# gmweir/PYFFT

Measured on AMD Instinct MI355X. Metric: Msamples/sec Welch-PSD 4096-pt Hann 50% overlap, complex64, higher is better.
Workload: dtype f32

## Files before the change

### pyfft_amd/csrc/fft_core.h

```cpp
#pragma once
#include <type_traits>
#include <hip/hip_runtime.h>

namespace sp {

typedef float2 cf;

__device__ __forceinline__ cf mk(float a, float b) { return make_float2(a, b); }
__device__ __forceinline__ cf operator+(cf a, cf b) { return mk(a.x + b.x, a.y + b.y); }
__device__ __forceinline__ cf operator-(cf a, cf b) { return mk(a.x - b.x, a.y - b.y); }
__device__ __forceinline__ cf operator*(float s, cf a) { return mk(s * a.x, s * a.y); }
__device__ __forceinline__ cf cmul(cf a, cf b) { return mk(a.x * b.x - a.y * b.y, a.x * b.y + a.y * b.x); }
__device__ __forceinline__ cf cmulc(cf a, cf b) { return mk(a.x * b.x + a.y * b.y, a.y * b.x - a.x * b.y); }
__device__ __forceinline__ cf cconj(cf a) { return mk(a.x, -a.y); }
__device__ __forceinline__ float cnorm(cf a) { return a.x * a.x + a.y * a.y; }

template <bool INV> __device__ __forceinline__ cf rot(cf a) { return INV ? mk(-a.y, a.x) : mk(a.y, -a.x); }
template <bool INV> __device__ __forceinline__ cf twc(cf a, float C, float S) {
    return INV ? mk(a.x * C - a.y * S, a.y * C + a.x * S) : mk(a.x * C + a.y * S, a.y * C - a.x * S);
}
template <bool INV> __device__ __forceinline__ cf twm(cf a, cf w) { return INV ? cmulc(a, w) : cmul(a, w); }

#define SP_C8 0.70710678118654752440f
#define SP_C16 0.92387953251128675613f
#define SP_S16 0.38268343236508977173f

template <bool INV> __device__ __forceinline__ void dft2(cf &a, cf &b) {
    cf t = a - b;
    a = a + b;
    b = t;
}

template <bool INV> __device__ __forceinline__ void dft4(cf &a, cf &b, cf &c, cf &d) {
    cf t0 = a + c, t1 = a - c, t2 = b + d, t3 = rot<INV>(b - d);
    a = t0 + t2;
    c = t0 - t2;
    b = t1 + t3;
    d = t1 - t3;
}

template <bool INV> __device__ __forceinline__ void dft8(cf (&x)[8]) {
    dft4<INV>(x[0], x[2], x[4], x[6]);
    dft4<INV>(x[1], x[3], x[5], x[7]);
    cf o1 = twc<INV>(x[3], SP_C8, SP_C8);
    cf o2 = rot<INV>(x[5]);
    cf o3 = twc<INV>(x[7], -SP_C8, SP_C8);
    cf e0 = x[0], e1 = x[2], e2 = x[4], e3 = x[6], o0 = x[1];
    x[0] = e0 + o0;
    x[4] = e0 - o0;
    x[1] = e1 + o1;
    x[5] = e1 - o1;
    x[2] = e2 + o2;
    x[6] = e2 - o2;
    x[3] = e3 + o3;
    x[7] = e3 - o3;
}

template <bool INV> __device__ __forceinline__ void dft16(cf (&x)[16]) {
#pragma unroll
    for (int b = 0; b < 4; ++b) dft4<INV>(x[b], x[b + 4], x[b + 8], x[b + 12]);
    x[5] = twc<INV>(x[5], SP_C16, SP_S16);
    x[9] = twc<INV>(x[9], SP_C8, SP_C8);
    x[13] = twc<INV>(x[13], SP_S16, SP_C16);
    x[6] = twc<INV>(x[6], SP_C8, SP_C8);
    x[10] = rot<INV>(x[10]);
    x[14] = twc<INV>(x[14], -SP_C8, SP_C8);
    x[7] = twc<INV>(x[7], SP_S16, SP_C16);
    x[11] = twc<INV>(x[11], -SP_C8, SP_C8);
    x[15] = twc<INV>(x[15], -SP_C16, -SP_S16);
#pragma unroll
    for (int c = 0; c < 4; ++c) dft4<INV>(x[4 * c], x[4 * c + 1], x[4 * c + 2], x[4 * c + 3]);
    cf t;
#define SP_SWAP(i, j) t = x[i]; x[i] = x[j]; x[j] = t;
    SP_SWAP(1, 4) SP_SWAP(2, 8) SP_SWAP(3, 12) SP_SWAP(6, 9) SP_SWAP(7, 13) SP_SWAP(11, 14)
#undef SP_SWAP
}

struct Tw16 {
    float f[40];
    static constexpr int TAU = 0, RB = 15, RC = 19, RD = 23, S1 = 27, S2 = 31, S3 = 35;
};

#define SP_T16 0.41421356237309504880f
#define SP_T316 2.41421356237309504880f

__device__ __forceinline__ void dft4s(cf &a, cf &b, cf &c, cf &d, float rb, float rc, float rd) {
    const cf t0 = mk(fmaf(rc, c.x, a.x), fmaf(rc, c.y, a.y));
    const cf t1 = mk(fmaf(-rc, c.x, a.x), fmaf(-rc, c.y, a.y));
    const cf t2 = mk(fmaf(rd, d.x, b.x), fmaf(rd, d.y, b.y));
    const cf t3 = mk(fmaf(-rd, d.x, b.x), fmaf(-rd, d.y, b.y));
    a = mk(fmaf(rb, t2.x, t0.x), fmaf(rb, t2.y, t0.y));
    c = mk(fmaf(-rb, t2.x, t0.x), fmaf(-rb, t2.y, t0.y));
    b = mk(fmaf(rb, t3.y, t1.x), fmaf(-rb, t3.x, t1.y));
    d = mk(fmaf(-rb, t3.y, t1.x), fmaf(rb, t3.x, t1.y));
}
__device__ __forceinline__ cf rot_tan(cf a, float t) { return mk(fmaf(t, a.y, a.x), fmaf(-t, a.x, a.y)); }

template <bool TWD, bool PREROT = false> __device__ __forceinline__ void dft16s(cf (&x)[16], const Tw16 &w) {
    if constexpr (TWD) {
        if constexpr (!PREROT) {
#pragma unroll
            for (int s = 1; s < 16; ++s) x[s] = rot_tan(x[s], w.f[Tw16::TAU + s - 1]);
        }
#pragma unroll
        for (int b = 0; b < 4; ++b) dft4s(x[b], x[b + 4], x[b + 8], x[b + 12], w.f[Tw16::RB + b], w.f[Tw16::RC + b], w.f[Tw16::RD + b]);
    } else {
#pragma unroll
        for (int b = 0; b < 4; ++b) dft4<false>(x[b], x[b + 4], x[b + 8], x[b + 12]);
    }
    x[5] = rot_tan(x[5], SP_T16);
    x[9] = mk(x[9].x + x[9].y, x[9].y - x[9].x);
    x[13] = rot_tan(x[13], SP_T316);
    x[6] = mk(x[6].x + x[6].y, x[6].y - x[6].x);
    x[10] = mk(x[10].y, -x[10].x);
    x[14] = mk(x[14].x - x[14].y, x[14].y + x[14].x);
    x[7] = rot_tan(x[7], SP_T316);
    x[11] = mk(x[11].x - x[11].y, x[11].y + x[11].x);
    x[15] = rot_tan(x[15], SP_T16);
    if constexpr (TWD) {
#pragma unroll
        for (int c = 0; c < 4; ++c) dft4s(x[4 * c], x[4 * c + 1], x[4 * c + 2], x[4 * c + 3], w.f[Tw16::S1 + c], w.f[Tw16::S2 + c], w.f[Tw16::S3 + c]);
    } else {
        dft4<false>(x[0], x[1], x[2], x[3]);
        dft4s(x[4], x[5], x[6], x[7], SP_C16, SP_C8, SP_S16 / SP_C16);
        dft4s(x[8], x[9], x[10], x[11], SP_C8, 1.f, -1.f);
        dft4s(x[12], x[13], x[14], x[15], SP_S16, -SP_C8, -SP_C16 / SP_S16);
    }
    cf t;
#define SP_SWAP(i, j) t = x[i]; x[i] = x[j]; x[j] = t;
    SP_SWAP(1, 4) SP_SWAP(2, 8) SP_SWAP(3, 12) SP_SWAP(6, 9) SP_SWAP(7, 13) SP_SWAP(11, 14)
#undef SP_SWAP
}

template <bool TWD, class Store, bool PREROT = false> __device__ __forceinline__ void dft16s_es(cf (&x)[16], const Tw16 &w, Store store) {
    if constexpr (TWD) {
        if constexpr (!PREROT) {
#pragma unroll
            for (int s = 1; s < 16; ++s) x[s] = rot_tan(x[s], w.f[Tw16::TAU + s - 1]);
        }
#pragma unroll
        for (int b = 0; b < 4; ++b) dft4s(x[b], x[b + 4], x[b + 8], x[b + 12], w.f[Tw16::RB + b], w.f[Tw16::RC + b], w.f[Tw16::RD + b]);
    } else {
#pragma unroll
        for (int b = 0; b < 4; ++b) dft4<false>(x[b], x[b + 4], x[b + 8], x[b + 12]);
    }
    x[5] = rot_tan(x[5], SP_T16);
    x[9] = mk(x[9].x + x[9].y, x[9].y - x[9].x);
    x[13] = rot_tan(x[13], SP_T316);
    x[6] = mk(x[6].x + x[6].y, x[6].y - x[6].x);
    x[10] = mk(x[10].y, -x[10].x);
    x[14] = mk(x[14].x - x[14].y, x[14].y + x[14].x);
    x[7] = rot_tan(x[7], SP_T316);
    x[11] = mk(x[11].x - x[11].y, x[11].y + x[11].x);
    x[15] = rot_tan(x[15], SP_T16);
    __builtin_amdgcn_sched_barrier(0);
#define SP_ES_OUT(c)                                                                                                 \
    store(c, x[4 * c]);                                                                                              \
    store(c + 4, x[4 * c + 1]);                                                                                      \
    store(c + 8, x[4 * c + 2]);                                                                                      \
    store(c + 12, x[4 * c + 3]);                                                                                     \
    __builtin_amdgcn_sched_barrier(0);
    if constexpr (TWD) {
        dft4s(x[0], x[1], x[2], x[3], w.f[Tw16::S1 + 0], w.f[Tw16::S2 + 0], w.f[Tw16::S3 + 0]);
        SP_ES_OUT(0)
        dft4s(x[4], x[5], x[6], x[7], w.f[Tw16::S1 + 1], w.f[Tw16::S2 + 1], w.f[Tw16::S3 + 1]);
        SP_ES_OUT(1)
        dft4s(x[8], x[9], x[10], x[11], w.f[Tw16::S1 + 2], w.f[Tw16::S2 + 2], w.f[Tw16::S3 + 2]);
        SP_ES_OUT(2)
        dft4s(x[12], x[13], x[14], x[15], w.f[Tw16::S1 + 3], w.f[Tw16::S2 + 3], w.f[Tw16::S3 + 3]);
        SP_ES_OUT(3)
    } else {
        dft4<false>(x[0], x[1], x[2], x[3]);
        SP_ES_OUT(0)
        dft4s(x[4], x[5], x[6], x[7], SP_C16, SP_C8, SP_S16 / SP_C16);
        SP_ES_OUT(1)
        dft4s(x[8], x[9], x[10], x[11], SP_C8, 1.f, -1.f);
        SP_ES_OUT(2)
        dft4s(x[12], x[13], x[14], x[15], SP_S16, -SP_C8, -SP_C16 / SP_S16);
        SP_ES_OUT(3)
    }
#undef SP_ES_OUT
}

__device__ __forceinline__ void dft4w(cf &a, cf &b, cf &c, cf &d, float wa, float wb, float wc, float wd) {
    const cf pa = mk(wa * a.x, wa * a.y), pb = mk(wb * b.x, wb * b.y);
    const cf t0 = mk(fmaf(wc, c.x, pa.x), fmaf(wc, c.y, pa.y));
    const cf t1 = mk(fmaf(-wc, c.x, pa.x), fmaf(-wc, c.y, pa.y));
    const cf t2 = mk(fmaf(wd, d.x, pb.x), fmaf(wd, d.y, pb.y));
    const cf t3 = mk(fmaf(-wd, d.x, pb.x), fmaf(-wd, d.y, pb.y));
    a = t0 + t2;
    c = t0 - t2;
    b = mk(t1.x + t3.y, t1.y - t3.x);
    d = mk(t1.x - t3.y, t1.y + t3.x);
}
struct NoMid {
    __device__ __forceinline__ void operator()(int) const {}
};
template <class Store, class Mid = NoMid> __device__ __forceinline__ void dft16s_es_win(cf (&x)[16], const float (&w)[16], Store store, Mid mid = Mid()) {
#pragma unroll
    for (int b = 0; b < 4; ++b) {
        dft4w(x[b], x[b + 4], x[b + 8], x[b + 12], w[b], w[b + 4], w[b + 8], w[b + 12]);
        if constexpr (!std::is_same<Mid, NoMid>::value) {
            if (b < 3) {
                __builtin_amdgcn_sched_barrier(0);
                mid(b);
                __builtin_amdgcn_sched_barrier(0);
            }
        }
    }
    x[5] = rot_tan(x[5], SP_T16);
    x[9] = mk(x[9].x + x[9].y, x[9].y - x[9].x);
    x[13] = rot_tan(x[13], SP_T316);
    x[6] = mk(x[6].x + x[6].y, x[6].y - x[6].x);
    x[10] = mk(x[10].y, -x[10].x);
    x[14] = mk(x[14].x - x[14].y, x[14].y + x[14].x);
    x[7] = rot_tan(x[7], SP_T316);
    x[11] = mk(x[11].x - x[11].y, x[11].y + x[11].x);
    x[15] = rot_tan(x[15], SP_T16);
    __builtin_amdgcn_sched_barrier(0);
#define SP_ES_OUT(c)                                                                                                 \
    store(c, x[4 * c]);                                                                                              \
    store(c + 4, x[4 * c + 1]);                                                                                      \
    store(c + 8, x[4 * c + 2]);                                                                                      \
    store(c + 12, x[4 * c + 3]);                                                                                     \
    __builtin_amdgcn_sched_barrier(0);
    dft4<false>(x[0], x[1], x[2], x[3]);
    SP_ES_OUT(0)
    dft4s(x[4], x[5], x[6], x[7], SP_C16, SP_C8, SP_S16 / SP_C16);
    SP_ES_OUT(1)
    dft4s(x[8], x[9], x[10], x[11], SP_C8, 1.f, -1.f);
    SP_ES_OUT(2)
    dft4s(x[12], x[13], x[14], x[15], SP_S16, -SP_C8, -SP_C16 / SP_S16);
    SP_ES_OUT(3)
#undef SP_ES_OUT
}

__device__ __forceinline__ void make_tw16(Tw16 &w, const cf (&wv)[15]) {
    float g[16];
    g[0] = 1.f;
    w.f[39] = 0.f;
#pragma unroll
    for (int s = 1; s < 16; ++s) {
        float c = wv[s - 1].x;
        if (fabsf(c) < 9.094947e-13f) c = c < 0.f ? -9.094947e-13f : 9.094947e-13f;
        g[s] = c;
        w.f[Tw16::TAU + s - 1] = -wv[s - 1].y / c;
    }
#pragma unroll
    for (int b = 0; b < 4; ++b) {
        w.f[Tw16::RB + b] = g[b + 4] / g[b];
        w.f[Tw16::RC + b] = g[b + 8] / g[b];
        w.f[Tw16::RD + b] = g[b + 12] / g[b + 4];
    }
    const float K1[4] = {1.f, SP_C16, SP_C8, SP_S16}, K2[4] = {1.f, SP_C8, 1.f, -SP_C8}, K3[4] = {1.f, SP_S16, -SP_C8, -SP_C16};
#pragma unroll
    for (int c = 0; c < 4; ++c) {
        w.f[Tw16::S1 + c] = g[1] * K1[c];
        w.f[Tw16::S2 + c] = g[2] * K2[c];
        w.f[Tw16::S3 + c] = (g[3] * K3[c]) / (g[1] * K1[c]);
    }
}

typedef float sp_f2v __attribute__((ext_vector_type(2)));
__device__ __forceinline__ cf lds_load_single(const cf *p) { return *p; }
template <int RDX, bool INV> __device__ __forceinline__ void dftR(cf (&x)[RDX]) {
    if constexpr (RDX == 2) dft2<INV>(x[0], x[1]);
    else if constexpr (RDX == 4) dft4<INV>(x[0], x[1], x[2], x[3]);
    else if constexpr (RDX == 8) dft8<INV>(x);
    else if constexpr (RDX == 16) dft16<INV>(x);
}

constexpr int ilog2c(int n) { return n <= 1 ? 0 : 1 + ilog2c(n >> 1); }

template <int N> struct FftPlan {
    static_assert(N >= 2 && (N & (N - 1)) == 0, "power of two");
    static constexpr int LOG2N = ilog2c(N);
    static constexpr int R = N < 16 ? N : 16;
    static constexpr int T = N / R;
    static constexpr int NP16 = N < 16 ? 0 : LOG2N / 4;
    static constexpr int REM = N < 16 ? N : (1 << (LOG2N % 4));
    static constexpr int NP = N < 16 ? 1 : NP16 + (REM > 1 ? 1 : 0);
    static constexpr int radix(int p) { return N < 16 ? N : (p < NP16 ? 16 : REM); }
    static constexpr int ns(int p) { int s = 1; for (int i = 0; i < p; ++i) s *= radix(i); return s; }
    static constexpr int ntw_before(int p) { int c = 0; for (int i = 1; i < p; ++i) c += (R / radix(i)) * (radix(i) - 1); return c; }
    static constexpr int NTW = ntw_before(NP);
    static constexpr int PITCH1 = T + 1;
    static constexpr int LDS_ELEMS = NP > 1 ? (R * PITCH1 > N ? R * PITCH1 : N) : 0;
};

#define SP_TW1_PITCH 44
template <int N, bool TW1LDS = false> struct WgFft {
    using PL = FftPlan<N>;
    static constexpr int R = PL::R, T = PL::T, NP = PL::NP;
    static constexpr int IMG0 = PL::LDS_ELEMS;
    static constexpr int N16 = PL::NP16 > 1 ? PL::NP16 - 1 : 0;
    static constexpr int NTR = (N >= 16 && PL::REM > 1) ? (R / PL::REM) * (PL::REM - 1) : 0;
    Tw16 t16[N16 > 0 ? N16 : 1];
    cf twr[NTR > 0 ? NTR : 1];
    const float *tw1 = nullptr;

    __device__ __forceinline__ void publish_tw1(float *table, int tid) {
        if constexpr (TW1LDS && N16 > 0) {
            if (tid < 16) {
#pragma unroll
                for (int j = 0; j < 40; ++j) table[tid * SP_TW1_PITCH + j] = t16[0].f[j];
            }
            tw1 = table;
        }
    }

    __device__ __forceinline__ void load_twiddles(const cf *__restrict__ table, int tid) {
        load_tw<1>(table, tid);
    }

    template <int P> __device__ __forceinline__ void load_tw(const cf *__restrict__ table, int tid) {
        if constexpr (P < NP) {
            constexpr int r = PL::radix(P), NS = PL::ns(P), NB = R / r;
            if constexpr (r == 16) {
                const int e = (tid % NS) * (N / (NS * 16));
                cf wv[15];
#pragma unroll
                for (int s = 1; s < 16; ++s) wv[s - 1] = table[e * s];
                make_tw16(t16[P - 1], wv);
            } else {
#pragma unroll
                for (int u = 0; u < NB; ++u) {
                    const int q = tid + T * u;
                    const int e = (q % NS) * (N / (NS * r));
#pragma unroll
                    for (int s = 1; s < r; ++s) twr[u * (r - 1) + (s - 1)] = table[e * s];
                }
            }
            load_tw<P + 1>(table, tid);
        }
    }

    template <int P> __device__ __forceinline__ void load_tw_one(const cf *__restrict__ table, int tid) {
        static_assert(P >= 1 && P < NP && PL::radix(P) == 16, "a twiddled radix-16 pass");
        constexpr int NS = PL::ns(P);
        const int e = (tid % NS) * (N / (NS * 16));
        cf wv[15];
#pragma unroll
        for (int s = 1; s < 16; ++s) wv[s - 1] = table[e * s];
        make_tw16(t16[P - 1], wv);
    }

    template <int E> static __device__ __forceinline__ int phys(int i) {
        if constexpr (E == 0) return (i % PL::radix(0)) * PL::PITCH1 + i / PL::radix(0);
        else return i;
    }

    template <int P> __device__ __forceinline__ void bfly(cf (&v)[R], int tid) const {
        constexpr int r = PL::radix(P), NB = R / r;
#pragma unroll
        for (int u = 0; u < NB; ++u) {
            cf x[r];
#pragma unroll
            for (int s = 0; s < r; ++s) x[s] = v[u + s * NB];
            if constexpr (r == 16) {
                if constexpr (TW1LDS && P == 1) {
                    Tw16 wl;
                    const float4 *row = reinterpret_cast<const float4 *>(tw1 + (tid % 16) * SP_TW1_PITCH);
#pragma unroll
                    for (int j = 0; j < 10; ++j) {
                        const float4 q = row[j];
                        wl.f[4 * j] = q.x;
                        wl.f[4 * j + 1] = q.y;
                        wl.f[4 * j + 2] = q.z;
                        wl.f[4 * j + 3] = q.w;
                    }
                    dft16s<true>(x, wl);
                } else if constexpr (P > 0) {
                    dft16s<true>(x, t16[P - 1]);
                } else {
                    dft16s<false>(x, t16[0]);
                }
            } else {
                if constexpr (P > 0) {
#pragma unroll
                    for (int s = 1; s < r; ++s) x[s] = twm<false>(x[s], twr[u * (r - 1) + (s - 1)]);
                }
                dftR<r, false>(x);
            }
#pragma unroll
            for (int s = 0; s < r; ++s) v[u + s * NB] = x[s];
        }
    }
    template <int P> __device__ __forceinline__ void scatter(const cf (&v)[R], cf *lds, int tid) const {
        constexpr int r = PL::radix(P), NS = PL::ns(P), NB = R / r;
#pragma unroll
        for (int u = 0; u < NB; ++u) {
            const int q = tid + T * u;
            const int base = (q / NS) * (NS * r) + (q % NS);
#pragma unroll
            for (int s = 0; s < r; ++s) lds[phys<P>(base + s * NS)] = v[u + s * NB];
        }
    }
    template <int P> __device__ __forceinline__ void gather(cf (&v)[R], const cf *lds, int tid) const {
        if constexpr (P == 0 && (T % 16) == 0 && PL::radix(0) == 16) {
            const int b = (tid % 16) * PL::PITCH1 + tid / 16;
#pragma unroll
            for (int t = 0; t < R; ++t) v[t] = lds_load_single(&lds[b + (T / 16) * t]);
        } else {
#pragma unroll
            for (int t = 0; t < R; ++t) v[t] = lds_load_single(&lds[phys<P>(tid + T * t)]);
        }
    }

    template <bool SINGLE, bool WL = false> __device__ __forceinline__ void run(cf (&v)[R], cf *lds0, cf *lds1, int tid) const {
        static_assert(!WL || T <= 64, "wave-local exchange: one wave holds the whole transform");
        pass<0, SINGLE, WL>(v, lds0, lds1, tid);
    }
    template <bool WL> static __device__ __forceinline__ void xsync() {
        if constexpr (WL) __builtin_amdgcn_wave_barrier();
        else __syncthreads();
    }

    template <int P> __device__ __forceinline__ void bfly_scatter(cf (&v)[R], cf *lds, int tid) const {
        constexpr int NS = PL::ns(P);
        const int base = (tid / NS) * (NS * 16) + (tid % NS);
        auto store = [&](int k, cf val) __attribute__((always_inline)) { lds[phys<P>(base + k * NS)] = val; };
        if constexpr (P > 0) dft16s_es<true>(v, t16[P - 1], store);
        else dft16s_es<false>(v, t16[0], store);
    }

    template <int P> __device__ __forceinline__ void load_tau_out(const cf *__restrict__ table, int tid, float (&tau)[16]) const {
        static_assert(P + 1 < NP && PL::radix(P) == 16 && PL::radix(P + 1) == 16 && R == 16, "between two radix-16 passes");
        constexpr int NS = PL::ns(P), NS2 = PL::ns(P + 1);
#pragma unroll
        for (int k = 0; k < 16; ++k) {
            const int p = (tid / NS) * (NS * 16) + (tid % NS) + k * NS;
            const int tc = p % T, sc = p / T;
            const int e = (tc % NS2) * (N / (NS2 * 16));
            const cf w = table[(e * sc) & (N - 1)];
            float c = w.x;
            if (fabsf(c) < 9.094947e-13f) c = c < 0.f ? -9.094947e-13f : 9.094947e-13f;
            tau[k] = sc == 0 ? 0.f : -w.y / c;
        }
    }
    template <int P, bool PREROT> __device__ __forceinline__ void bfly_scatter_rot(cf (&v)[R], const float (&tau)[16], cf *lds, int tid) const {
        constexpr int NS = PL::ns(P);
        const int base = (tid / NS) * (NS * 16) + (tid % NS);
        auto store = [&](int k, cf val) __attribute__((always_inline)) { lds[phys<P>(base + k * NS)] = rot_tan(val, tau[k]); };
        if constexpr (P > 0) dft16s_es<true, decltype(store), PREROT>(v, t16[P - 1], store);
        else dft16s_es<false>(v, t16[0], store);
    }
    __device__ __forceinline__ void bfly_scatter_win_rot(cf (&v)[R], const float (&w)[R], const float (&tau)[16], cf *lds, int tid) const {
        static_assert(R == 16, "radix-16 first pass");
        constexpr int NS = PL::ns(0);
        const int base = (tid / NS) * (NS * 16) + (tid % NS);
        auto store = [&](int k, cf val) __attribute__((always_inline)) { lds[phys<0>(base + k * NS)] = rot_tan(val, tau[k]); };
        dft16s_es_win(v, w, store);
    }
    template <int P> __device__ __forceinline__ void bfly_prerot(cf (&v)[R], int tid) const {
        (void)tid;
        static_assert(P > 0 && PL::radix(P) == 16 && R == 16, "a twiddled radix-16 pass");
        dft16s<true, true>(v, t16[P - 1]);
    }

    __device__ __forceinline__ void bfly_scatter_win(cf (&v)[R], const float (&w)[R], cf *lds, int tid) const {
        static_assert(R == 16, "radix-16 first pass");
        constexpr int NS = PL::ns(0);
        const int base = (tid / NS) * (NS * 16) + (tid % NS);
        auto store = [&](int k, cf val) __attribute__((always_inline)) { lds[phys<0>(base + k * NS)] = val; };
        dft16s_es_win(v, w, store);
    }

    template <int P, bool SINGLE, bool WL = false> __device__ __forceinline__ void pass(cf (&v)[R], cf *lds0, cf *lds1, int tid) const {
        constexpr bool LAST = (P == NP - 1);
        cf *lds = (P & 1) ? lds1 : lds0;
        if constexpr (!LAST && SINGLE) xsync<WL>();
        bfly<P>(v, tid);
        if constexpr (!LAST) {
            scatter<P>(v, lds, tid);
            xsync<WL>();
            gather<P>(v, lds, tid);
            pass<P + 1, SINGLE, WL>(v, lds0, lds1, tid);
        }
    }
};

}
```

### pyfft_amd/csrc/k_welch_pipe.hip

```cpp
#include "launch.h"
#include <type_traits>
#define SP_PIPE_AHEAD 2
namespace sp {

template <bool CPLX, int SHIFT, int MODE>
__global__ __launch_bounds__(768) void k_welch_pipe(const void *__restrict__ x_in, const float *__restrict__ win,
                                                     int64_t nframes, int64_t fpg, float *__restrict__ trend_in, XfTables tb,
                                                     float *__restrict__ partial, cf *__restrict__ spartial, int64_t x_cs, int gpr) {
    constexpr int N = 4096;
    constexpr bool RP = MODE >= 3 && MODE != 8 && MODE != 9;
    constexpr bool ONEPASS = MODE == 1 || MODE == 4 || MODE == 7 || MODE == 8 || MODE == 9, COG = MODE == 2 || MODE == 8;
    constexpr bool LOBE = MODE == 9;
    constexpr bool SPEC = MODE == 5 || MODE == 7;
    const void *x = SPEC ? (const void *)(reinterpret_cast<const float *>(x_in) + (int64_t)blockIdx.y * x_cs) : x_in;
    float *trend = SPEC ? trend_in + 4 * blockIdx.y : trend_in;
    static_assert(!RP || (!CPLX && SHIFT == 8), "the real-pair form is for real input at hop = nfft / 2");
    using PL = FftPlan<N>;
    using F = WgFft<N>;
    constexpr int T = PL::T, R = PL::R, KEEP = R - SHIFT, IMG = F::IMG0, IMGB = PL::LDS_ELEMS;
    static_assert(T == 256 && R == 16 && PL::NP == 3, "three radix-16 passes over 256 threads");
    extern __shared__ __attribute__((aligned(16))) unsigned char smem_raw[];
    cf *smem = reinterpret_cast<cf *>(smem_raw);
    cf *imgA = smem, *imgB = smem + 2 * IMG;
    const int role = __builtin_amdgcn_readfirstlane((int)threadIdx.x >> 8);
    const int tid = (int)threadIdx.x & 255;
    const int hop = SHIFT * T;

    cf mu;
    if constexpr (ONEPASS) {
        const int64_t span = (nframes - 1) * (int64_t)hop + N;
        const int64_t pitch = span / 16;
        constexpr int NU = SPEC ? 4 : 1, NTH = SPEC ? 3 * T : T, NWV = SPEC ? 12 : 4;
        const int lt = SPEC ? (int)threadIdx.x : tid;
        float sx = 0.f, sy = 0.f;
#pragma unroll
        for (int r = 0; r < 16; ++r)
#pragma unroll
            for (int u = 0; u < NU; ++u) {
                int64_t i = pitch * r + (int64_t)(lt + NTH * u);
                i = i < span ? i : span - 1;
                const cf v = load_sample(x, i, CPLX);
                sx += v.x;
                sy += v.y;
            }
        sx = wave_sum64(sx);
        sy = wave_sum64(sy);
        float *red = reinterpret_cast<float *>(smem);
        if ((SPEC || role == 0) && (tid & 63) == 0) {
            red[2 * (lt >> 6)] = sx;
            red[2 * (lt >> 6) + 1] = sy;
        }
        __syncthreads();
        double tx = 0.0, ty = 0.0;
#pragma unroll
        for (int wv = 0; wv < NWV; ++wv) {
            tx += (double)red[2 * wv];
            ty += (double)red[2 * wv + 1];
        }
        mu = mk((float)(tx / (16.0 * NTH * NU)), (float)(ty / (16.0 * NTH * NU)));
        __syncthreads();
        if (blockIdx.x == 0 && threadIdx.x == 0) {
            trend[0] = mu.x;
            trend[1] = mu.y;
            trend[2] = 0.f;
            trend[3] = 0.f;
        }
    } else {
        mu = load_trend(trend).m;
    }
    const int64_t gid = blockIdx.x;
    const int64_t g0 = gid * fpg;
    const int64_t last = nframes - 1;
    int64_t trips = (RP ? (nframes + 1) / 2 : nframes) - g0;
    trips = trips < 0 ? 0 : (trips > fpg ? fpg : trips);
    constexpr int DRAIN = 4;
    const int64_t periods = trips + DRAIN;
    F f;
    constexpr bool UPROT = !RP;
    float tau_out[16];
    if constexpr (UPROT) {
        if (role == 0) f.template load_tau_out<0>(tb.tw, tid, tau_out);
        else if (role == 1) f.template load_tau_out<1>(tb.tw, tid, tau_out);
    }

    if (role == 0 && RP) {
        const float *xr = reinterpret_cast<const float *>(x);
        float m = mu.x;
        asm volatile("" : "+v"(m));
        float w[R], sacc[SHIFT];
#pragma unroll
        for (int t = 0; t < R; ++t) w[t] = win[tid + T * t];
#pragma unroll
        for (int s = 0; s < SHIFT; ++s) sacc[s] = 0.f;
        auto issue_chunk = [&](float (&dst)[R], int64_t q) __attribute__((always_inline)) {
            const int64_t q1 = 2 * q <= nframes ? q : 0, q2 = 2 * q + 1 <= nframes ? q : 0;
            const float *b1 = xr + q1 * (int64_t)N, *b2 = xr + q2 * (int64_t)N;
#pragma unroll
            for (int t = 0; t < R; ++t) {
                const unsigned off = (unsigned)(tid + T * t);
                dst[t] = __builtin_nontemporal_load((t < R / 2 ? b1 : b2) + off);
            }
        };
        float ca[R], cb[R], cc[R];
        issue_chunk(ca, g0);
        issue_chunk(cb, g0 + 1);
#pragma unroll
        for (int t = 0; t < R; ++t) {
            ca[t] -= m;
            cb[t] -= m;
        }
        auto frame = [&](auto hb, int64_t i, cf *img, float (&cur)[R], float (&nxt)[R], float (&fill)[R]) __attribute__((always_inline)) {
            constexpr bool HB = decltype(hb)::value;
            issue_chunk(fill, g0 + i + 2);
            __builtin_amdgcn_sched_barrier(0);
            cf v[R];
            if constexpr (!ONEPASS) {
#pragma unroll
                for (int t = 0; t < R; ++t) v[t] = mk(cur[t], HB ? (t < R / 2 ? cur[t + R / 2] : nxt[t - R / 2]) : 0.f);
                if constexpr (UPROT) f.bfly_scatter_win_rot(v, w, tau_out, img, tid);
                else f.bfly_scatter_win(v, w, img, tid);
            } else {
#pragma unroll
                for (int t = 0; t < R; ++t) v[t] = mk(w[t] * cur[t], HB ? w[t] * (t < R / 2 ? cur[t + R / 2] : nxt[t - R / 2]) : 0.f);
                if constexpr (UPROT) f.template bfly_scatter_rot<0, false>(v, tau_out, img, tid);
                else f.template bfly_scatter<0>(v, img, tid);
            }
            __builtin_amdgcn_sched_barrier(0);
            if constexpr (ONEPASS) {
#pragma unroll
                for (int s = 0; s < SHIFT; ++s) sacc[s] += HB ? cur[R / 2 + s] + nxt[s] : cur[R / 2 + s];
            }
#pragma unroll
            for (int t = 0; t < R; ++t) fill[t] -= m;
        };
        const std::true_type yes;
        const std::false_type no;
        int64_t i = 0;
        for (; i + 6 < trips; i += 6) {
            frame(yes, i, imgA, ca, cb, cc);
            __syncthreads();
            frame(yes, i + 1, imgA + IMG, cb, cc, ca);
            __syncthreads();
            frame(yes, i + 2, imgA, cc, ca, cb);
            __syncthreads();
            frame(yes, i + 3, imgA + IMG, ca, cb, cc);
            __syncthreads();
            frame(yes, i + 4, imgA, cb, cc, ca);
            __syncthreads();
            frame(yes, i + 5, imgA + IMG, cc, ca, cb);
            __syncthreads();
        }
        for (; i < trips; ++i) {
            cf *img = (i & 1) ? imgA + IMG : imgA;
            const bool has_b = 2 * (g0 + i) + 1 < nframes;
            if (has_b) {
                if (i % 3 == 0) frame(yes, i, img, ca, cb, cc);
                else if (i % 3 == 1) frame(yes, i, img, cb, cc, ca);
                else frame(yes, i, img, cc, ca, cb);
            } else {
                if (i % 3 == 0) frame(no, i, img, ca, cb, cc);
                else if (i % 3 == 1) frame(no, i, img, cb, cc, ca);
                else frame(no, i, img, cc, ca, cb);
            }
            __syncthreads();
        }
#pragma unroll
        for (int d = 0; d < DRAIN; ++d) __syncthreads();
        if constexpr (ONEPASS) {
#pragma unroll
            for (int s = 0; s < SHIFT; ++s)
                spartial[((SPEC ? (int64_t)blockIdx.y * gridDim.x : 0) + gid) * hop + tid + T * s] = mk(sacc[s], 0.f);
        }
    } else if (role == 0) {
        asm volatile("" : "+v"(mu.x), "+v"(mu.y));
        float w[R];
        cf sacc[SHIFT], raw[R];
#pragma unroll
        for (int t = 0; t < R; ++t) w[t] = win[tid + T * t];
#pragma unroll
        for (int s = 0; s < SHIFT; ++s) sacc[s] = mk(0.f, 0.f);
        {
            const int64_t base = (g0 < nframes ? g0 : last) * hop + tid;
#pragma unroll
            for (int t = 0; t < R; ++t) raw[t] = load_sample(x, base + T * t, CPLX) - mu;
        }
        auto issue_part = [&](cf (&dst)[SHIFT], int64_t q, int s0, int s1) __attribute__((always_inline)) {
            const int64_t gq = g0 + q;
            const int64_t gn = gq < nframes ? gq : last;
            const int64_t ubase = gn * hop + (int64_t)T * KEEP;
#pragma unroll
            for (int s = s0; s < s1; ++s) {
                const unsigned off = (unsigned)(tid + T * s);
                if (CPLX) {
                    const sp_f2v r = __builtin_nontemporal_load(reinterpret_cast<const sp_f2v *>(x) + ubase + off);
                    dst[s] = mk(r.x, r.y);
                } else {
                    dst[s] = mk(__builtin_nontemporal_load(reinterpret_cast<const float *>(x) + ubase + off), 0.f);
                }
            }
        };
        auto issue = [&](cf (&dst)[SHIFT], int64_t q) __attribute__((always_inline)) { issue_part(dst, q, 0, SHIFT); };
        constexpr int AHEAD = (SP_PIPE_AHEAD >= 2 && SHIFT <= 8) ? (SP_PIPE_AHEAD >= 3 ? 3 : 2) : 1;
        constexpr bool SPREAD = AHEAD >= 2;
        auto frame = [&](int64_t i, cf *img, cf (&fill)[SHIFT], cf (&take)[SHIFT]) __attribute__((always_inline)) {
            if constexpr (SPREAD) issue_part(fill, i + AHEAD, 0, SHIFT / 4);
            else issue(fill, i + AHEAD);
            __builtin_amdgcn_sched_barrier(0);
            cf v[R];
            constexpr bool WINFOLD = SPREAD;
#pragma unroll
            for (int t = 0; t < R; ++t) v[t] = WINFOLD ? raw[t] : w[t] * raw[t];
            if constexpr (SPREAD) {
            {
                auto store = [&](int k, cf val) __attribute__((always_inline)) {
                    img[F::template phys<0>(tid * 16 + k)] = UPROT ? rot_tan(val, tau_out[k]) : val;
                    if (k >= 12 && k < 15) issue_part(fill, i + AHEAD, (k - 11) * (SHIFT / 4), (k - 10) * (SHIFT / 4));
                };
                if constexpr (WINFOLD) dft16s_es_win(v, w, store);
                else dft16s_es<false>(v, f.t16[0], store);
            }
            } else {
            if constexpr (UPROT) f.template bfly_scatter_rot<0, false>(v, tau_out, img, tid);
            else f.template bfly_scatter<0>(v, img, tid);
            }
            __builtin_amdgcn_sched_barrier(0);
#pragma unroll
            for (int s = 0; s < SHIFT; ++s)
                if constexpr (ONEPASS && !LOBE) sacc[s] = sacc[s] + raw[KEEP + s];
#pragma unroll
            for (int t = 0; t < KEEP; ++t) raw[t] = raw[t + SHIFT];
#pragma unroll
            for (int s = 0; s < SHIFT; ++s) raw[KEEP + s] = take[s] - mu;
        };
        int64_t i = 0;
        if constexpr (AHEAD == 3) {
            cf s0[SHIFT], s1[SHIFT], s2[SHIFT];
            issue(s1, 1);
            issue(s2, 2);
            for (; i + 2 < trips; i += 3) {
                frame(i, (i & 1) ? imgA + IMG : imgA, s0, s1);
                __syncthreads();
                frame(i + 1, ((i + 1) & 1) ? imgA + IMG : imgA, s1, s2);
                __syncthreads();
                frame(i + 2, ((i + 2) & 1) ? imgA + IMG : imgA, s2, s0);
                __syncthreads();
            }
            for (; i < trips; ++i) {
                cf *img = (i & 1) ? imgA + IMG : imgA;
                if (i % 3 == 0) frame(i, img, s0, s1);
                else if (i % 3 == 1) frame(i, img, s1, s2);
                else frame(i, img, s2, s0);
                __syncthreads();
            }
        } else if constexpr (AHEAD == 2) {
            cf nxa[SHIFT], nxb[SHIFT];
            issue(nxa, 1);
            for (; i + 1 < trips; i += 2) {
                frame(i, imgA, nxb, nxa);
                __syncthreads();
                frame(i + 1, imgA + IMG, nxa, nxb);
                __syncthreads();
            }
            if (i < trips) {
                frame(i, imgA, nxb, nxa);
                __syncthreads();
            }
        } else {
            for (; i + 1 < trips; i += 2) {
                cf nx0[SHIFT], nx1[SHIFT];
                frame(i, imgA, nx0, nx0);
                __syncthreads();
                frame(i + 1, imgA + IMG, nx1, nx1);
                __syncthreads();
            }
            if (i < trips) {
                cf nx0[SHIFT];
                frame(i, imgA, nx0, nx0);
                __syncthreads();
            }
        }
#pragma unroll
        for (int d = 0; d < DRAIN; ++d) __syncthreads();
#pragma unroll
        for (int s = 0; s < SHIFT; ++s)
            if constexpr (ONEPASS && !LOBE) spartial[gid * hop + tid + T * s] = sacc[s];
    } else if (role == 1) {
        f.template load_tw_one<1>(tb.tw, tid);
        cf va[R], vb[R];
        auto step = [&](cf (&fill)[R], cf (&use)[R], int64_t p, const cf *src, cf *dst) __attribute__((always_inline)) {
            if (p >= 1 && p <= trips) f.template gather<0>(fill, src, tid);
            if (p >= 2 && p <= trips + 1) {
                if constexpr (UPROT) f.template bfly_scatter_rot<1, true>(use, tau_out, dst, tid);
                else f.template bfly_scatter<1>(use, dst, tid);
            }
            __syncthreads();
        };
        for (int64_t p = 0; p < periods; p += 2) {
            step(va, vb, p, imgA + IMG, imgB);
            if (p + 1 < periods) step(vb, va, p + 1, imgA, imgB + IMGB);
        }
    } else {
        f.template load_tw_one<2>(tb.tw, tid);
        float acc[R];
#pragma unroll
        for (int t = 0; t < R; ++t) acc[t] = 0.f;
        cf bs_lo = mk(0.f, 0.f), bs_hi = mk(0.f, 0.f);
        const unsigned zlo = (unsigned)((tid >> 3) * 512 + (tid & 7));
        cf held[SPEC ? R : 1];
        cf va[R], vb[R];
        cf pend = mk(0.f, 0.f);
        auto flush = [&](int64_t i) __attribute__((always_inline)) {
            const int sel = (int)(i & 63), li = tid & 63;
            const int64_t gg = g0 + (i - sel) + li;
            if (li <= sel && gg < nframes) reinterpret_cast<cf *>(partial)[(int64_t)(tid >> 6) * nframes + gg] = pend;
        };
        auto step = [&](cf (&fill)[R], cf (&use)[R], int64_t p, const cf *src) __attribute__((always_inline)) {
            if (p >= 3 && p <= trips + 2) {
                f.template gather<1>(fill, src, tid);
            }
            if (p >= 4 && p <= trips + 3) {
                if constexpr (UPROT) f.template bfly_prerot<2>(use, tid);
                else f.template bfly<2>(use, tid);
                if constexpr (SPEC) {
                    const int64_t pr = g0 + (p - 4);
                    const bool lone = (pr & 1) == 0 && p == trips + 3;
                    if ((pr & 1) == 0 && !lone) {
#pragma unroll
                        for (int t = 0; t < R; ++t) held[t] = use[t];
                    } else {
                        float4 *zb = reinterpret_cast<float4 *>(partial) + ((pr >> 1) * (int64_t)gpr * 512 + (int64_t)blockIdx.y * 8);
                        unsigned bl = zlo;
                        asm volatile("" : "+v"(bl));
#pragma unroll
                        for (int t = 0; t < R; ++t) {
                            const float4 q = lone ? make_float4(use[t].x, use[t].y, 0.f, 0.f)
                                                  : make_float4(held[t].x, held[t].y, use[t].x, use[t].y);
                            st_stream(zb + (bl + 16384u * t), q);
                        }
                    }
                } else if constexpr (COG) {
                    if constexpr (MODE == 8) {
                        const int64_t gf = g0 + (p - 4);
                        cf *lobe = reinterpret_cast<cf *>(partial) + 4 * nframes + gf * 8;
                        if (gf < nframes) {
                            if (tid <= 3) lobe[3 + tid] = use[0];
                            if (tid >= T - 3) lobe[3 - (T - tid)] = use[R - 1];
                        }
                    }
                    float numc = 0.f, den = 0.f;
#pragma unroll
                    for (int t = 0; t < R; ++t) {
                        const float pw = cnorm(use[t]);
                        numc = fmaf(pw, (float)(T * t - (t >= R / 2 ? N : 0)), numc);
                        den += pw;
                    }
                    float num = fmaf((float)tid, den, numc);
                    num = wave_sum64(num);
                    den = wave_sum64(den);
                    const int64_t i = p - 4;
                    if ((tid & 63) == (int)(i & 63)) pend = mk(num, den);
                    if ((i & 63) == 63 || i == trips - 1) flush(i);
                } else {
#pragma unroll
                    for (int t = 0; t < R; ++t) acc[t] = fmaf(use[t].y, use[t].y, fmaf(use[t].x, use[t].x, acc[t]));
                    if constexpr (LOBE) {
                        bs_lo = bs_lo + use[0];
                        bs_hi = bs_hi + use[R - 1];
                    }
                }
            }
            __syncthreads();
        };
        for (int64_t p = 0; p < periods; p += 2) {
            step(va, vb, p, imgB + IMGB);
            if (p + 1 < periods) step(vb, va, p + 1, imgB);
        }
        if constexpr (!COG && !SPEC) {
#pragma unroll
            for (int t = 0; t < R; ++t) partial[gid * N + tid + T * t] = acc[t];
            if constexpr (LOBE) {
                if (tid <= 3) spartial[gid * 8 + 3 + tid] = bs_lo;
                if (tid >= T - 3) spartial[gid * 8 + 3 - (T - tid)] = bs_hi;
                if (tid == 4) spartial[gid * 8 + 7] = mk(0.f, 0.f);
            }
        }
    }
}

bool welch_pipe_eligible(const Xf &xf, int hop) {
    return !xf.blue && xf.L == 4096 && (hop == 2048 || hop == 1024 || hop == 4096);
}

int launch_welch_pipe(LaunchCtx c, const void *x, bool cplx, const float *win, int hop, int64_t nframes, float *trend,
                      const Xf &xf, float *partial, const RunPart &rp, cf *spartial, int mode, int nch, int64_t x_cs, int gpr) {
    const size_t lds = sizeof(cf) * 4 * (size_t)FftPlan<4096>::LDS_ELEMS;
#define PIPE_(CP, S, OP)                                                                                  \
    {                                                                                                 \
        static bool once = false;                                                                     \
        if (!once) {                                                                                  \
            if (hipFuncSetAttribute((const void *)k_welch_pipe<CP, S, OP>, hipFuncAttributeMaxDynamicSharedMemorySize, (int)lds) != hipSuccess) \
                return -1;                                                                            \
            once = true;                                                                              \
        }                                                                                             \
        if (c.stop)                                                                                   \
            hipExtLaunchKernelGGL((k_welch_pipe<CP, S, OP>), dim3(rp.blocks, gy), dim3(768), lds, c.stream, nullptr, c.stop, 0, x, win, \
                                  nframes, rp.fpg, trend, xf.tb, partial, spartial, x_cs, gpr);       \
        else                                                                                          \
            hipLaunchKernelGGL((k_welch_pipe<CP, S, OP>), dim3(rp.blocks, gy), dim3(768), lds, c.stream, x, win, nframes, rp.fpg, trend, \
                               xf.tb, partial, spartial, x_cs, gpr);                                  \
    }
    const int shift = hop / 256;
    const unsigned gy = mode == 5 ? (unsigned)nch : 1u;
#define PIPE_S_(CP, OP)                                                                               \
    if (shift == 8) PIPE_(CP, 8, OP) else if (shift == 4) PIPE_(CP, 4, OP) else PIPE_(CP, 16, OP)
    if (mode == 5) {
        if (cplx || shift != 8 || nch < 1 || gpr < 1) return -1;
        if (spartial) PIPE_(false, 8, 7) else PIPE_(false, 8, 5)
    } else if (mode == 3) {
        if (cplx || shift != 8) return -1;
        if (spartial) PIPE_(false, 8, 4) else PIPE_(false, 8, 3)
    } else if (mode == 2 && spartial) {
        if (shift == 8) { if (cplx) PIPE_(true, 8, 8) else PIPE_(false, 8, 8) }
        else if (shift == 4) { if (cplx) PIPE_(true, 4, 8) else PIPE_(false, 4, 8) }
        else return -1;
    } else if (mode == 2) {
        if (cplx) { PIPE_S_(true, 2) } else { PIPE_S_(false, 2) }
    } else if (mode == 9) {
        if (!spartial || shift == 16) return -1;
        if (shift == 8) { if (cplx) PIPE_(true, 8, 9) else PIPE_(false, 8, 9) }
        else { if (cplx) PIPE_(true, 4, 9) else PIPE_(false, 4, 9) }
    } else if (spartial) {
        if (cplx) { PIPE_S_(true, 1) } else { PIPE_S_(false, 1) }
    } else {
        if (cplx) { PIPE_S_(true, 0) } else { PIPE_S_(false, 0) }
    }
#undef PIPE_S_
#undef PIPE_
    return 0;
}

}
```

Before: 481,800.

## Overlap one-pass mean estimate with first frame loads and batch its sample loads

For one-pass complex/non-real-pair modes, the mean estimate now runs after the producer role has issued its first frame and look-ahead loads, so that global-memory latency overlaps. The other two roles call the estimate after loading their twiddles, and the mean is subtracted from the raw frame afterwards. The estimate's sample loads are batched in groups of eight with scheduling barriers so more loads are in flight. A SEL template flag also reshapes the tau division select. This adds register pressure from holding the raw frame and look-ahead buffers during the reduction.

```diff
diff --git a/pyfft_amd/csrc/fft_core.h b/pyfft_amd/csrc/fft_core.h
--- a/pyfft_amd/csrc/fft_core.h
+++ b/pyfft_amd/csrc/fft_core.h
@@ -424,7 +424,7 @@
         else dft16s_es<false>(v, t16[0], store);
     }
 
-    template <int P> __device__ __forceinline__ void load_tau_out(const cf *__restrict__ table, int tid, float (&tau)[16]) const {
+    template <int P, bool SEL = true> __device__ __forceinline__ void load_tau_out(const cf *__restrict__ table, int tid, float (&tau)[16]) const {
         static_assert(P + 1 < NP && PL::radix(P) == 16 && PL::radix(P + 1) == 16 && R == 16, "between two radix-16 passes");
         constexpr int NS = PL::ns(P), NS2 = PL::ns(P + 1);
 #pragma unroll
@@ -435,7 +435,12 @@
             const cf w = table[(e * sc) & (N - 1)];
             float c = w.x;
             if (fabsf(c) < 9.094947e-13f) c = c < 0.f ? -9.094947e-13f : 9.094947e-13f;
-            tau[k] = sc == 0 ? 0.f : -w.y / c;
+            if constexpr (SEL) {
+                const float q = -w.y / c;
+                tau[k] = sc == 0 ? 0.f : q;
+            } else {
+                tau[k] = sc == 0 ? 0.f : -w.y / c;
+            }
         }
     }
     template <int P, bool PREROT> __device__ __forceinline__ void bfly_scatter_rot(cf (&v)[R], const float (&tau)[16], cf *lds, int tid) const {
diff --git a/pyfft_amd/csrc/k_welch_pipe.hip b/pyfft_amd/csrc/k_welch_pipe.hip
--- a/pyfft_amd/csrc/k_welch_pipe.hip
+++ b/pyfft_amd/csrc/k_welch_pipe.hip
@@ -26,23 +26,31 @@
     const int tid = (int)threadIdx.x & 255;
     const int hop = SHIFT * T;
 
-    cf mu;
-    if constexpr (ONEPASS) {
+    auto estimate_mu0 = [&]() __attribute__((always_inline)) -> cf {
         const int64_t span = (nframes - 1) * (int64_t)hop + N;
         const int64_t pitch = span / 16;
         constexpr int NU = SPEC ? 4 : 1, NTH = SPEC ? 3 * T : T, NWV = SPEC ? 12 : 4;
         const int lt = SPEC ? (int)threadIdx.x : tid;
         float sx = 0.f, sy = 0.f;
-#pragma unroll
-        for (int r = 0; r < 16; ++r)
-#pragma unroll
-            for (int u = 0; u < NU; ++u) {
+        constexpr int EB = SHIFT > 8 ? 1 : 8;
+#pragma unroll
+        for (int b = 0; b < 16 * NU / EB; ++b) {
+            cf v[EB];
+#pragma unroll
+            for (int j = 0; j < EB; ++j) {
+                const int r = (EB * b + j) / NU, u = (EB * b + j) % NU;
                 int64_t i = pitch * r + (int64_t)(lt + NTH * u);
                 i = i < span ? i : span - 1;
-                const cf v = load_sample(x, i, CPLX);
-                sx += v.x;
-                sy += v.y;
-            }
+                v[j] = load_sample(x, i, CPLX);
+            }
+            __builtin_amdgcn_sched_barrier(0);
+#pragma unroll
+            for (int j = 0; j < EB; ++j) {
+                sx += v[j].x;
+                sy += v[j].y;
+            }
+            __builtin_amdgcn_sched_barrier(0);
+        }
         sx = wave_sum64(sx);
         sy = wave_sum64(sy);
         float *red = reinterpret_cast<float *>(smem);
@@ -57,17 +65,20 @@
             tx += (double)red[2 * wv];
             ty += (double)red[2 * wv + 1];
         }
-        mu = mk((float)(tx / (16.0 * NTH * NU)), (float)(ty / (16.0 * NTH * NU)));
+        const cf m0 = mk((float)(tx / (16.0 * NTH * NU)), (float)(ty / (16.0 * NTH * NU)));
         __syncthreads();
         if (blockIdx.x == 0 && threadIdx.x == 0) {
-            trend[0] = mu.x;
-            trend[1] = mu.y;
+            trend[0] = m0.x;
+            trend[1] = m0.y;
             trend[2] = 0.f;
             trend[3] = 0.f;
         }
-    } else {
-        mu = load_trend(trend).m;
-    }
+        return m0;
+    };
+    constexpr bool EARLY = ONEPASS && !RP && SHIFT <= 8;
+    cf mu = mk(0.f, 0.f);
+    if constexpr (!ONEPASS) mu = load_trend(trend).m;
+    else if constexpr (!EARLY) mu = estimate_mu0();
     const int64_t gid = blockIdx.x;
     const int64_t g0 = gid * fpg;
     const int64_t last = nframes - 1;
@@ -79,14 +90,13 @@
     constexpr bool UPROT = !RP;
     float tau_out[16];
     if constexpr (UPROT) {
-        if (role == 0) f.template load_tau_out<0>(tb.tw, tid, tau_out);
-        else if (role == 1) f.template load_tau_out<1>(tb.tw, tid, tau_out);
+        constexpr bool SEL = !(ONEPASS && SHIFT > 8);
+        if (role == 0) f.template load_tau_out<0, SEL>(tb.tw, tid, tau_out);
+        else if (role == 1) f.template load_tau_out<1, SEL>(tb.tw, tid, tau_out);
     }
 
     if (role == 0 && RP) {
         const float *xr = reinterpret_cast<const float *>(x);
-        float m = mu.x;
-        asm volatile("" : "+v"(m));
         float w[R], sacc[SHIFT];
 #pragma unroll
         for (int t = 0; t < R; ++t) w[t] = win[tid + T * t];
@@ -104,6 +114,8 @@
         float ca[R], cb[R], cc[R];
         issue_chunk(ca, g0);
         issue_chunk(cb, g0 + 1);
+        float m = mu.x;
+        asm volatile("" : "+v"(m));
 #pragma unroll
         for (int t = 0; t < R; ++t) {
             ca[t] -= m;
@@ -172,7 +184,6 @@
                 spartial[((SPEC ? (int64_t)blockIdx.y * gridDim.x : 0) + gid) * hop + tid + T * s] = mk(sacc[s], 0.f);
         }
     } else if (role == 0) {
-        asm volatile("" : "+v"(mu.x), "+v"(mu.y));
         float w[R];
         cf sacc[SHIFT], raw[R];
 #pragma unroll
@@ -182,7 +193,10 @@
         {
             const int64_t base = (g0 < nframes ? g0 : last) * hop + tid;
 #pragma unroll
-            for (int t = 0; t < R; ++t) raw[t] = load_sample(x, base + T * t, CPLX) - mu;
+            for (int t = 0; t < R; ++t) {
+                raw[t] = load_sample(x, base + T * t, CPLX);
+                if constexpr (!EARLY) raw[t] = raw[t] - mu;
+            }
         }
         auto issue_part = [&](cf (&dst)[SHIFT], int64_t q, int s0, int s1) __attribute__((always_inline)) {
             const int64_t gq = g0 + q;
@@ -202,6 +216,17 @@
         auto issue = [&](cf (&dst)[SHIFT], int64_t q) __attribute__((always_inline)) { issue_part(dst, q, 0, SHIFT); };
         constexpr int AHEAD = (SP_PIPE_AHEAD >= 2 && SHIFT <= 8) ? (SP_PIPE_AHEAD >= 3 ? 3 : 2) : 1;
         constexpr bool SPREAD = AHEAD >= 2;
+        cf nxa[AHEAD == 2 ? SHIFT : 1], nxb[AHEAD == 2 ? SHIFT : 1];
+        if constexpr (AHEAD == 2) issue(nxa, 1);
+        if constexpr (EARLY) {
+            __builtin_amdgcn_sched_barrier(0);
+            mu = estimate_mu0();
+        }
+        asm volatile("" : "+v"(mu.x), "+v"(mu.y));
+        if constexpr (EARLY) {
+#pragma unroll
+            for (int t = 0; t < R; ++t) raw[t] = raw[t] - mu;
+        }
         auto frame = [&](int64_t i, cf *img, cf (&fill)[SHIFT], cf (&take)[SHIFT]) __attribute__((always_inline)) {
             if constexpr (SPREAD) issue_part(fill, i + AHEAD, 0, SHIFT / 4);
             else issue(fill, i + AHEAD);
@@ -253,8 +278,6 @@
                 __syncthreads();
             }
         } else if constexpr (AHEAD == 2) {
-            cf nxa[SHIFT], nxb[SHIFT];
-            issue(nxa, 1);
             for (; i + 1 < trips; i += 2) {
                 frame(i, imgA, nxb, nxa);
                 __syncthreads();
@@ -286,6 +309,10 @@
             if constexpr (ONEPASS && !LOBE) spartial[gid * hop + tid + T * s] = sacc[s];
     } else if (role == 1) {
         f.template load_tw_one<1>(tb.tw, tid);
+        if constexpr (EARLY) {
+            __builtin_amdgcn_sched_barrier(0);
+            (void)estimate_mu0();
+        }
         cf va[R], vb[R];
         auto step = [&](cf (&fill)[R], cf (&use)[R], int64_t p, const cf *src, cf *dst) __attribute__((always_inline)) {
             if (p >= 1 && p <= trips) f.template gather<0>(fill, src, tid);
@@ -301,6 +328,10 @@
         }
     } else {
         f.template load_tw_one<2>(tb.tw, tid);
+        if constexpr (EARLY) {
+            __builtin_amdgcn_sched_barrier(0);
+            (void)estimate_mu0();
+        }
         float acc[R];
 #pragma unroll
         for (int t = 0; t < R; ++t) acc[t] = 0.f;
```

Measured after the change: 477,200. Within noise of the previous version (-0.9%).
